# ictnlp/StreamSpeech

Hardware: AMD Instinct MI355X
Metric: real-time factor (RTFx = audio seconds / wall seconds) + utterances/sec, offline S2ST fr-en (higher is better)
Workload: dtype f32

## Files before the change

### include/streamspeech_hip.h

```cpp
#ifndef STREAMSPEECH_HIP_H
#define STREAMSPEECH_HIP_H

#include <stddef.h>
#include <stdint.h>

#ifdef __cplusplus
extern "C" {
#endif

#define SS_ABI_VERSION 2

typedef struct ss_model ss_model;
typedef struct ss_vocoder ss_vocoder;
typedef struct ss_scratch ss_scratch;
typedef struct ss_stream_pool ss_stream_pool;

typedef struct ss_config {
  int32_t input_feat, conv_channels, conv_kernel;
  int32_t enc_dim, enc_ffn, enc_heads, enc_layers, dw_kernel;
  int32_t src_vocab, tgt_vocab;
  int32_t mt_layers, dec_dim, dec_ffn, dec_heads;
  int32_t t2u_layers, unit_layers, unit_vocab, ctc_upsample;
  int32_t pad, eos, unk;
  int32_t max_rel_pos;
// ... 416 lines not shown
                 double* h_bytes_total);
int ss_prof_totals(int cls, double* h_flops_total, double* h_bytes_total, int64_t* h_launches);
int ss_prof_read_issued(int cls, double* h_issued_flops_total);
int ss_prof_shape_log(int on);
int ss_prof_shape_dump(char* buf, int cap);
int ss_prof_num_classes(void);
const char* ss_prof_class_name(int cls);

int ss_model_set_pack_invariant(ss_model* m, int on);
int ss_model_get_pack_invariant(ss_model* m);
int ss_debug_canon(int mode);

int ss_debug_last_logits(ss_model* m, void* stream, float* d_out, int64_t cap_floats, int* h_rows, int* h_cols);

int ss_op_ffn_fused(void* stream, const float* dX, int ldx, float* dY, int ldy, const float* ln_g, const float* ln_b,
                    const float* dW1, const float* db1, const float* dW2, const float* db2, float alpha,
                    const float* ln2_g, const float* ln2_b, int M, int D, int F);
int ss_debug_ffn(int grid, int row_tiles_per_wave, int enable);
int ss_debug_rtlin(int grid, int enable);
int ss_debug_rtlin_kb(int uw, int order);
int ss_debug_rtlin_kb_last(int32_t out[4]);
int ss_debug_conv_c64(int enable);
int ss_debug_conv_c256_rows(int rows);
int ss_debug_conv_c32(int enable);
int ss_debug_conv_c16(int enable);
int64_t ss_debug_enc_step_launches(void);
int ss_op_ln_linear(void* stream, const float* dX, int ldx, const float* ln_g, const float* ln_b, const float* dW,
                    const float* dbias, const float* dR, int ldr, float* dC, int ldc, int M, int N, int K, int act, float alpha,
                    int glu);
int ss_op_ln_linear_ex(void* stream, const float* dX, int ldx, const float* ln_g, const float* ln_b, float* ln_out, const float* dW,
                       const float* dbias, const float* dR, int ldr, float* dC, int ldc, int M, int N, int K, int act, float alpha,
                       int glu, int canon);

int ss_debug_force_tile(int bm, int bn, int ks);
int ss_debug_sk_errors(void);
int ss_debug_attention_split(int v);
int ss_debug_attention_q16(int v);
int ss_debug_enc_step_inject_timeout(ss_model* m);
int ss_debug_scratch_audit(ss_scratch* sc, size_t* booked, size_t* held);
int ss_debug_mt_inject_timeout(ss_model* m);

int ss_op_conv_gemm(void* stream, const float* dA, int lda, const float* dW, const float* dbias,
                    const float* dR, int ldr, const float* dR2, int ldr2, float* dC, int ldc,
                    int M, int N, int Cin, int taps, int dil, int stride, int pad, int in_len,
                    int chunk, int in_act, float in_slope, int act, float alpha, float div, int glu);
typedef struct ss_op_conv_args {
// ... 143 lines not shown
```

### streamspeech_amd/csrc/debug_ops.hip

```cpp
#include "model_internal.hpp"
#include "ctc_align.hpp"

static int op_bind_wino(GemmArgs& a, void* stream) {
  static thread_local std::map<hipStream_t, DevBuf> wino_tmps;
  DevBuf& wino_tmp = wino_tmps[(hipStream_t)stream];
  const int N = a.N, Cin = a.Cin, taps = a.taps;
  if ((conv_c64w_enabled() && N == 64 && Cin == 64 && taps >= 3 && conv_c64_eligible(a)) ||
      (conv_c128w_enabled() && N == 128 && Cin == 128 && taps >= 3 && a.same_rows && !a.glu) ||
      (conv_c256w_enabled() && N == 256 && Cin == 256 && taps >= 3 && a.same_rows && !a.glu) ||
      (conv_c32w_enabled() && N == 32 && Cin == 32 && taps >= 3 && conv_c32_eligible(a))) {
    RET(wino_tmp.ensure((size_t)N * ((taps + 2) / 3) * 4 * N * sizeof(float)));
    RET(launch_wino_pack(a.W, wino_tmp.f(), N, taps, (hipStream_t)stream));
    a.Wwino = wino_tmp.f();
  }
  return SS_OK;
}

extern "C" int ss_op_conv_gemm(void* stream, const float* dA, int lda, const float* dW, const float* dbias,
                               const float* dR, int ldr, const float* dR2, int ldr2, float* dC, int ldc, int M,
                               int N, int Cin, int taps, int dil, int stride, int pad, int in_len, int chunk,
                               int in_act, float in_slope, int act, float alpha, float div, int glu) {
  GemmArgs a;
  a.A = dA; a.lda = lda; a.W = dW; a.bias = dbias; a.R = dR; a.ldr = ldr; a.R2 = dR2; a.ldr2 = ldr2; a.C = dC; a.ldc = ldc;
  a.M = M; a.N = N; a.Cin = Cin; a.taps = taps; a.dil = dil; a.stride = stride; a.pad = pad; a.in_len = in_len;
// ... 95 lines not shown
  a.A = dX; a.lda = ldx; a.W = dW; a.bias = dbias; a.R = dR; a.ldr = ldr; a.C = dC; a.ldc = ldc;
  a.M = M; a.N = N; a.Cin = K; a.in_len = M; a.act = act; a.alpha = alpha; a.glu = glu; a.same_rows = 1;
  a.ln_g = ln_g; a.ln_b = ln_b;
  return launch_conv_gemm(a, (hipStream_t)stream);
}
extern "C" int ss_op_ln_linear_ex(void* stream, const float* dX, int ldx, const float* ln_g, const float* ln_b, float* ln_out,
                                  const float* dW, const float* dbias, const float* dR, int ldr, float* dC, int ldc, int M, int N, int K,
                                  int act, float alpha, int glu, int canon) {
  if (canon < 0 || canon > 2 || (ln_g == nullptr) != (ln_b == nullptr) || (ln_out && !ln_g)) return SS_ERR_ARG;
  GemmArgs a;
  a.A = dX; a.lda = ldx; a.W = dW; a.bias = dbias; a.R = dR; a.ldr = ldr; a.C = dC; a.ldc = ldc;
  a.M = M; a.N = N; a.Cin = K; a.in_len = M; a.act = act; a.alpha = alpha; a.glu = glu; a.same_rows = 1;
  a.ln_g = ln_g; a.ln_b = ln_b; a.ln_out = ln_out; a.canon = canon;
  return launch_conv_gemm(a, (hipStream_t)stream);
}
extern "C" int ss_debug_conv_c64(int enable) {
  if (enable == 4 || enable == 5) { conv_c64w_debug(enable == 5); return SS_OK; }
  if (enable == 6 || enable == 7) { conv_c128w_debug(enable == 7); return SS_OK; }
  if (enable == 8 || enable == 9) { conv_c256w_debug(enable == 9); return SS_OK; }
  conv_c64_debug(enable);
  return SS_OK;
}
extern "C" int ss_debug_conv_c256_rows(int rows) { return conv_c256w_rows_debug(rows); }
extern "C" int ss_debug_conv_c32(int enable) {
  if (enable == 4 || enable == 5) { conv_c32w_debug(enable == 5); return SS_OK; }
  conv_c32_debug(enable);
  return SS_OK;
}
extern "C" int ss_debug_conv_c16(int enable) { conv_c16_debug(enable); return SS_OK; }
extern "C" int64_t ss_debug_enc_step_launches(void) { return (int64_t)enc_step_launch_count(); }
extern "C" int ss_debug_scratch_audit(ss_scratch* sc, size_t* booked, size_t* held) {
  if (!sc || !booked || !held) return SS_ERR_ARG;
  size_t sum = 0;
  bool foreign = false;
  for (DevBuf* b : sc->all()) {
    sum += b->bytes;
    if (b->acct != &sc->acct) foreign = true;
  }
  *booked = sc->acct.used;
  *held = sum;
  return foreign ? SS_ERR_ARG : SS_OK;
}
extern "C" int ss_debug_rtlin(int grid, int enable) {
  if (grid < 0) return SS_ERR_ARG;
  rtlin_debug(grid, enable);
  return SS_OK;
// ... 211 lines not shown
```

### streamspeech_amd/csrc/dispatch.hip

```cpp
#include "gemm.hpp"

#include <atomic>
#include <cstdlib>
#include <map>
#include <mutex>
#include <utility>
#include <vector>

namespace ss {

namespace {
std::mutex g_disp_mu;
std::atomic<unsigned> g_disp_gen{1};
Dispatch env_defaults() {
  Dispatch d;
  auto I = [](const char* k, int dflt) { const char* e = getenv(k); return e ? atoi(e) : dflt; };
  auto L = [](const char* k, long long dflt) { const char* e = getenv(k); return e ? atoll(e) : dflt; };
  d.attn_split = I("SS_ATTN_NO_SPLIT", 0) ? -1 : 0; d.attn_q16 = I("SS_ATTN_Q16", d.attn_q16);
  d.c16_off = I("SS_NO_CONV_C16", 0) ? 1 : 0; d.c32_off = I("SS_NO_CONV_C32", 0) ? 1 : 0; d.c64_off = I("SS_NO_CONV_C64", 0) ? 1 : 0;
  d.c16_min_rows = L("SS_CONV_C16_MIN_ROWS", d.c16_min_rows); d.c32_min_rows = L("SS_CONV_C32_MIN_ROWS", d.c32_min_rows);
  d.c64_min_rows = L("SS_CONV_C64_MIN_ROWS", d.c64_min_rows);
  d.c64w_on = I("SS_CONV_C64_WINOGRAD", 1); d.c128w_on = I("SS_CONV_C128_WINOGRAD", 1); d.c256w_on = I("SS_CONV_C256_WINOGRAD", 1);
  d.c32w_on = I("SS_CONV_C32_WINOGRAD", 1); d.c64w_min_k = I("SS_CONV_C64_WINOGRAD_MIN_K", 3);
  d.c128w_min_rows = L("SS_CONV_C128_MIN_ROWS", d.c128w_min_rows); d.c256w_min_rows = L("SS_CONV_C256_MIN_ROWS", d.c256w_min_rows);
  if (const int r = I("SS_CONV_C256_ROWS", d.c256w_rows); r == 128 || r == 256) d.c256w_rows = r;
  if (getenv("SS_FFN_WM")) { d.ffn_wm = I("SS_FFN_WM", 3); d.ffn_wm_forced = 1; d.ffn_wm_env = d.ffn_wm; }
  d.ffn_fusion = I("SS_NO_FFN_FUSION", 0) ? 0 : 1; d.ffn_min_rows = I("SS_FFN_MIN_ROWS", d.ffn_min_rows);
  if (getenv("SS_SK_MIN_GFLOP")) d.sk_min_flops = 1e9 * atof(getenv("SS_SK_MIN_GFLOP"));
  d.no_resblock_fusion = I("SS_NO_RESBLOCK_FUSION", 0); d.no_pair_fusion = I("SS_NO_PAIR_FUSION", 0);
  d.rt_off = I("SS_NO_RTLIN", 0) ? 1 : 0; d.rt_min_rows = I("SS_RTLIN_MIN_ROWS", d.rt_min_rows); d.rt_min_units = L("SS_RTLIN_MIN_UNITS", d.rt_min_units);
  d.rt_kb_min_units = L("SS_RTLIN_KB_MIN_UNITS", d.rt_kb_min_units); d.rt_kb_uw = I("SS_RTLIN_KB_UW", d.rt_kb_uw); d.rt_kb_xmap = I("SS_RTLIN_KB_XMAP", d.rt_kb_xmap);
  d.smallm_max_rows = I("SS_SMALLM_MAX_ROWS", d.smallm_max_rows); d.sk_min_units = L("SS_SK_MIN_UNITS", d.sk_min_units);
  d.no_sk2 = I("SS_NO_SK2", 0) ? 1 : 0; d.sk2_min_k64 = I("SS_SK2_MINK64", d.sk2_min_k64); d.sk2_spare_cus = I("SS_SK2_SPARE_CUS", 0);
  d.rt_wg_per_cu = I("SS_RTLIN_WG_PER_CU", 0); d.c32_min_k = I("SS_CONV_C32_MIN_K", d.c32_min_k); d.c16_min_k = I("SS_CONV_C16_MIN_K", d.c16_min_k);
  return d;
}
Dispatch& process_settings() { static Dispatch d = env_defaults(); return d; }
thread_local const Dispatch* t_disp = nullptr;
thread_local CtxDispatch t_disp_own;
}
void dispatch_edit(const std::function<void(Dispatch&)>& fn) {
  std::lock_guard<std::mutex> lk(g_disp_mu);
  fn(process_settings());
  g_disp_gen.fetch_add(1, std::memory_order_release);
}
void slab_debug(int grid, long long min_rows) {
  const Dispatch dflt = env_defaults();
  dispatch_edit([=](Dispatch& d) {
    d.slab_grid_cap = grid > 0 ? grid : 0;
    const bool set = min_rows >= 0;
    d.c16_min_rows = set ? min_rows : dflt.c16_min_rows; d.c32_min_rows = set ? min_rows : dflt.c32_min_rows;
    d.c64_min_rows = set ? min_rows : dflt.c64_min_rows;
    d.c128w_min_rows = set ? min_rows : dflt.c128w_min_rows; d.c256w_min_rows = set ? min_rows : dflt.c256w_min_rows;
  });
}
int conv_c256w_rows_debug(int rows) {
  if (rows != 0 && rows != 128 && rows != 256) return SS_ERR_ARG;
  const int dflt = env_defaults().c256w_rows;
  dispatch_edit([=](Dispatch& d) { d.c256w_rows = rows ? rows : dflt; });
  return SS_OK;
}
const Dispatch* CtxDispatch::refresh() {
  const unsigned now = g_disp_gen.load(std::memory_order_acquire);
  if (gen != now) {
    std::lock_guard<std::mutex> lk(g_disp_mu);
    d = process_settings();
    gen = g_disp_gen.load(std::memory_order_relaxed);
  }
  return &d;
}
const Dispatch& disp() { return t_disp ? *t_disp : *t_disp_own.refresh(); }
DispatchScope::DispatchScope(const Dispatch* d) : prev(t_disp) { t_disp = d; }
DispatchScope::~DispatchScope() { t_disp = prev; }

void debug_force_tile(int bm, int bn, int ks) {
  dispatch_edit([=](Dispatch& d) { d.force_bm = bm; d.force_bn = bn; d.force_ks = ks; d.sk_groups = (bm == 1 && bn == 8); });
}
bool debug_tile_forced() { return disp().force_bm != 0; }

static thread_local int t_canon = CANON_NONE;
CanonScope::CanonScope(int mode) : prev(t_canon) { t_canon = mode; }
CanonScope::~CanonScope() { t_canon = prev; }
// ... 93 lines not shown
```

### streamspeech_amd/csrc/dispatch.hpp

```cpp
#pragma once
#include <functional>

namespace ss {

struct Dispatch {
  int attn_no_mfma = 0;
  int attn_q16 = 1;
  int attn_split = 0;
  int c16_off = 0, c32_off = 0, c64_off = 0;
  long long c16_min_rows = 131072, c32_min_rows = 65536, c64_min_rows = 32768;
  int c64w_on = 1, c128w_on = 1, c256w_on = 1, c32w_on = 1;
  int c64w_min_k = 3;
  long long c128w_min_rows = 65536, c256w_min_rows = 32768;
  int c256w_rows = 128;
  int c32_min_k = 7, c16_min_k = 11;
  int slab_grid_cap = 0;
  int sk_groups = 0;
  int sk2_spare_cus = 0;
  int ffn_force_g = 0;
  int ffn_wm = 3, ffn_wm_forced = 0;
  int ffn_wm_env = 0;
  int ffn_fusion = 1;
  int ffn_min_rows = 1000;
  int force_bm = 0, force_bn = 0, force_ks = 0;
  double sk_min_flops = 4e9;
  int smallm_max_rows = 192;
  long long sk_min_units = 12 * 512;
  int no_sk2 = 0;
  int sk2_min_k64 = 192;
  int no_resblock_fusion = 0, no_pair_fusion = 0;
  int rt_off = 0, rt_min_rows = 193, rt_force_g = 0;
  long long rt_min_units = 4000;
  int rt_wg_per_cu = 0;
  long long rt_kb_min_units = 256;
  int rt_kb_xmap = 1;
  int rt_kb_uw = 0;
  int rt_kb_order = 1;
};

const Dispatch& disp();
void dispatch_edit(const std::function<void(Dispatch&)>& fn);

struct CtxDispatch {
  Dispatch d;
  unsigned gen = 0xffffffffu;
  const Dispatch* refresh();
};
struct DispatchScope {
  explicit DispatchScope(const Dispatch* d);
// ... 6 lines not shown
```

### streamspeech_amd/csrc/gemm.hip

```cpp
#include "gemm.hpp"

#include <type_traits>

namespace ss {

using f32x4 = __attribute__((ext_vector_type(4))) float;

template <int BM, int BN, int BK, int WM, int WN, int KS, int PD, bool BLK = false>
__global__ __launch_bounds__(256 * KS) void conv_gemm_kernel(const GemmArgs p) {
  static_assert(WM * WN == 4, "4 waves per k-group");
  static_assert(!BLK || KS == 1, "the blocked chain is the KS = 1 form");
  constexpr int LDK = BK + 8;
  constexpr int WTM = BM / WM, WTN = BN / WN;
  constexpr int TM = WTM / 16, TN = WTN / 16;
  static_assert(TM >= 1 && TN >= 1, "wave tile must hold a 16x16 MFMA tile");
  constexpr int KQ = BK / 4;
  constexpr int A_F4 = BM * KQ, W_F4 = BN * KQ;
  constexpr int NA = (A_F4 + 255) / 256, NW = (W_F4 + 255) / 256;
  constexpr int STAGE = (BM + BN) * LDK;
  extern __shared__ __attribute__((aligned(16))) float smem_all[];
  const int kg = threadIdx.x >> 8;
  float* smem = smem_all + kg * 2 * STAGE;

  const int t = threadIdx.x & 255, lane = t & 63, wave = t >> 6;
// ... 269 lines not shown
          if (p.R2) x = p.R2[row * p.ldr2 + n + e] + x;
          if (p.div > 0.f) x = x / p.div;
          p.C[row * p.ldc + n + e] = x;
          if (p.C2) p.C2[row * p.ldc2 + n + e] = x > 0.f ? x : x * p.c2_slope;
        }
      }
    }
  }
}


__device__ __forceinline__ void linear_store(const GemmArgs& p, int m, int n, float acc, float b) {
  float v = acc + b;
  switch (p.act) {
    case ACT_SILU: v = v / (1.0f + expf(-v)); break;
    case ACT_RELU: v = fmaxf(v, 0.f); break;
    default: break;
  }
  v *= p.alpha;
  if (p.R) v += p.R[(size_t)m * p.ldr + n];
  p.C[(size_t)m * p.ldc + n] = v;
}

template <int SK, int WN, bool LNORM, bool GLU = false>
__global__ __launch_bounds__(256) void smallm_gemm_kernel(const GemmArgs p) {
  static_assert(SK * WN == 4, "4 waves");
  static_assert(!GLU || (SK == 2 && WN == 2), "GLU: wave column 0 = the 16 value columns, 1 = the 16 gate columns of a 32-column block");
  __shared__ f32x4 red[SK > 1 ? (SK - 1) * WN * 64 : 1];
  __shared__ float ln_stat[32];
  const int t = threadIdx.x, lane = t & 63, wave = t >> 6;
  const int sk = wave / WN, wn = wave % WN;
  const int r = lane & 15, g = lane >> 4;
  if ((int)blockIdx.x * (16 * WN) >= p.N) return;
  const int m0 = blockIdx.y * 16;
  const int n0 = blockIdx.x * (16 * WN) + wn * 16;
  const int K = p.Cin;
  const int KC = K / 16;
  const int c_begin = (KC * sk) / SK, c_end = (KC * (sk + 1)) / SK;

  const int am = m0 + r;
  const bool a_ok = am < p.M;
  const float* arow = p.A + (size_t)(a_ok ? am : 0) * p.lda + 4 * g;
  const int wnr = n0 + r;
  const bool w_ok = wnr < p.N;
  const float* wrow = p.W + (size_t)(w_ok ? wnr : 0) * K + 4 * g;

  float mean = 0.f, rstd = 1.f;
  if (LNORM) {
    const int lr = t >> 4, part = t & 15;
    const bool ok = (m0 + lr) < p.M;
    const float* xr = p.A + (size_t)(ok ? m0 + lr : 0) * p.lda + part * 4;
    f32x4 v[8];
    float sm = 0.f;
#pragma unroll
    for (int j = 0; j < 8; ++j) {
      v[j] = f32x4{0.f, 0.f, 0.f, 0.f};
      if (j * 64 < K && ok) v[j] = *reinterpret_cast<const f32x4*>(xr + j * 64);
      sm += (v[j][0] + v[j][1]) + (v[j][2] + v[j][3]);
    }
#pragma unroll
    for (int o = 1; o < 16; o <<= 1) sm += __shfl_xor(sm, o, 64);
    const float mu = sm / (float)K;
    float q = 0.f;
#pragma unroll
    for (int j = 0; j < 8; ++j)
      if (j * 64 < K) {
#pragma unroll
        for (int e = 0; e < 4; ++e) { const float d = v[j][e] - mu; q += d * d; }
      }
#pragma unroll
    for (int o = 1; o < 16; o <<= 1) q += __shfl_xor(q, o, 64);
    if (part == 0) { ln_stat[lr] = mu; ln_stat[16 + lr] = 1.0f / sqrtf(q / (float)K + 1e-5f); }
    __syncthreads();
    mean = ln_stat[r];
    rstd = ln_stat[16 + r];
  }

  f32x4 acc = {0.f, 0.f, 0.f, 0.f}, acc2 = {0.f, 0.f, 0.f, 0.f};
  f32x4 tot = {0.f, 0.f, 0.f, 0.f};
  const bool blocked = (c_end - c_begin) > 8;
  auto load4 = [&](f32x4 (&a)[4], f32x4 (&w)[4], int c) {
#pragma unroll
    for (int u = 0; u < 4; ++u) {
      a[u] = f32x4{0.f, 0.f, 0.f, 0.f};
      w[u] = f32x4{0.f, 0.f, 0.f, 0.f};
      if (a_ok) a[u] = *reinterpret_cast<const f32x4*>(arow + (c + u) * 16);
      if (w_ok) w[u] = *reinterpret_cast<const f32x4*>(wrow + (c + u) * 16);
    }
  };
  auto mma = [&](f32x4 a, f32x4 w, int c) {
    if (LNORM) {
      const f32x4 gm = *reinterpret_cast<const f32x4*>(p.ln_g + c * 16 + 4 * g);
      const f32x4 bt = *reinterpret_cast<const f32x4*>(p.ln_b + c * 16 + 4 * g);
#pragma unroll
      for (int e = 0; e < 4; ++e) a[e] = a_ok ? (a[e] - mean) * rstd * gm[e] + bt[e] : 0.f;
    }
    acc = __builtin_amdgcn_mfma_f32_16x16x4f32(a[0], w[0], acc, 0, 0, 0);
    acc2 = __builtin_amdgcn_mfma_f32_16x16x4f32(a[1], w[1], acc2, 0, 0, 0);
    acc = __builtin_amdgcn_mfma_f32_16x16x4f32(a[2], w[2], acc, 0, 0, 0);
    acc2 = __builtin_amdgcn_mfma_f32_16x16x4f32(a[3], w[3], acc2, 0, 0, 0);
    if (blocked && (c & 3) == 3) {
#pragma unroll
      for (int e = 0; e < 4; ++e) { tot[e] += acc[e] + acc2[e]; acc[e] = 0.f; acc2[e] = 0.f; }
    }
  };
  auto mma4 = [&](f32x4 (&a)[4], f32x4 (&w)[4], int c) {
#pragma unroll
    for (int u = 0; u < 4; ++u) mma(a[u], w[u], c + u);
  };
  const int G = (c_end - c_begin) / 4;
  f32x4 a0[4], w0[4], a1[4], w1[4];
  if (G > 0) load4(a0, w0, c_begin);
  for (int gi = 0; gi < G; gi += 2) {
    const int c = c_begin + 4 * gi;
    if (gi + 1 < G) load4(a1, w1, c + 4);
    mma4(a0, w0, c);
    if (gi + 1 < G) {
      if (gi + 2 < G) load4(a0, w0, c + 8);
      mma4(a1, w1, c + 4);
    }
  }
  for (int c = c_begin + 4 * G; c < c_end; ++c) {
    f32x4 a = {0.f, 0.f, 0.f, 0.f}, w = {0.f, 0.f, 0.f, 0.f};
    if (a_ok) a = *reinterpret_cast<const f32x4*>(arow + c * 16);
    if (w_ok) w = *reinterpret_cast<const f32x4*>(wrow + c * 16);
    mma(a, w, c);
  }
#pragma unroll
  for (int e = 0; e < 4; ++e) acc[e] = tot[e] + (acc[e] + acc2[e]);

  if (SK > 1) {
    if (sk > 0) red[((sk - 1) * WN + wn) * 64 + lane] = acc;
    __syncthreads();
    if (!GLU && sk > 0) return;
    if (sk == 0) {
#pragma unroll
      for (int s2 = 1; s2 < SK; ++s2) {
        const f32x4 o = red[((s2 - 1) * WN + wn) * 64 + lane];
#pragma unroll
        for (int e = 0; e < 4; ++e) acc[e] += o[e];
      }
    }
  }
  if constexpr (GLU) {
    __shared__ f32x4 gate_tile[64];
    const int ncol = n0 + r;
    const float bcol = (p.bias && ncol < p.N) ? p.bias[ncol] : 0.f;
    if (sk == 0 && wn == 1) {
      f32x4 gt;
#pragma unroll
      for (int e = 0; e < 4; ++e) gt[e] = acc[e] + bcol;
      gate_tile[lane] = gt;
    }
    __syncthreads();
    if (sk != 0 || wn != 0 || ncol + 16 >= p.N) return;
    const f32x4 gt = gate_tile[lane];
    const int oc = (int)blockIdx.x * 16 + r;
#pragma unroll
    for (int e = 0; e < 4; ++e) {
      const int m = m0 + g * 4 + e;
      if (m < p.M) p.C[(size_t)m * p.ldc + oc] = (acc[e] + bcol) * (1.0f / (1.0f + expf(-gt[e])));
    }
    return;
  }
  const int n = n0 + r;
  if (n >= p.N) return;
  const float b = p.bias ? p.bias[n] : 0.f;
#pragma unroll
  for (int e = 0; e < 4; ++e) {
    const int m = m0 + g * 4 + e;
    if (m < p.M) linear_store(p, m, n, acc[e], b);
  }
}


template <int MR, int KS, bool LNORM>
__global__ __launch_bounds__(256) void gemv_kernel(const GemmArgs p) {
  constexpr int WPB = 4;
  constexpr int CPB = WPB / KS;
  __shared__ float part[WPB][MR];
  const int t = threadIdx.x, lane = t & 63, wave = t >> 6;
  const int col = blockIdx.x * CPB + wave / KS;
  const int ks = wave % KS;
  const int K = p.Cin;
  const int kper = K / KS;
  const int k0 = ks * kper;
  const int nit = kper / 256;
  const bool col_ok = col < p.N;

  f32x4 wv[8];
  const float* wrow = p.W + (size_t)(col_ok ? col : 0) * K + k0 + 4 * lane;
#pragma unroll
  for (int it = 0; it < 8; ++it) {
    wv[it] = f32x4{0.f, 0.f, 0.f, 0.f};
    if (it < nit && col_ok) wv[it] = *reinterpret_cast<const f32x4*>(wrow + it * 256);
// ... 95 lines not shown
  static_assert((size_t)(KS - 1) * BM * BN * sizeof(float) <= kLds, "reduction scratch fits the staging buffers");
  if constexpr (kLds > 64 * 1024) SS_MAX_LDS_ONCE((&conv_gemm_kernel<BM, BN, BK, WM, WN, KS, PD, BLK>), kLds);
  const int mmax = (a.nseg > 0 ? a.max_seg_out : a.M) - a.m_begin;
  dim3 grid(cdiv(mmax, BM), cdiv(a.N, BN), a.nseg > 0 ? a.nseg : 1);
  if (grid.x >= 32 && grid.y * grid.z > 1) grid.x = (grid.x + 7) & ~7u;
  ProfRec rec{}; bool prof = false;
  int rc = prof_begin(a, stream, cls, rec, prof);
  if (rc != SS_OK) return rc;
  hipLaunchKernelGGL((conv_gemm_kernel<BM, BN, BK, WM, WN, KS, PD, BLK>), grid, dim3(256 * KS), kLds, stream, a);
  SS_LAUNCH_CHECK();
  return prof_end(stream, rec, prof);
}

template <int BM, int BN, int BK, int WM, int WN, int MAXKS>
static int launch_cfg_ks(const GemmArgs& a, hipStream_t stream, ProfCls cls, long tiles) {
  const int nk = a.taps * (a.Cin / BK);
  int ks = 1;
  while (ks < MAXKS && tiles * 4 * ks < 1024 && nk / (ks * 2) >= 2) ks *= 2;
  if constexpr (MAXKS >= 4) { if (ks >= 4) return launch_cfg<BM, BN, BK, WM, WN, 4>(a, stream, cls); }
  if constexpr (MAXKS >= 2) { if (ks >= 2) return launch_cfg<BM, BN, BK, WM, WN, 2>(a, stream, cls); }
  return launch_cfg<BM, BN, BK, WM, WN, 1>(a, stream, cls);
}

template <int SK, int WN, bool GLU = false>
static int launch_smallm(const GemmArgs& a, hipStream_t stream, ProfCls cls) {
  if (a.ln_g && a.Cin > 512) return SS_ERR_ARG;
  dim3 grid((cdiv(a.N, 16 * WN) + 7) & ~7, cdiv(a.M, 16));
  ProfRec rec{}; bool prof = false;
  int rc = prof_begin(a, stream, cls, rec, prof);
  if (rc != SS_OK) return rc;
  if (a.ln_g) hipLaunchKernelGGL((smallm_gemm_kernel<SK, WN, true, GLU>), grid, dim3(256), 0, stream, a);
  else hipLaunchKernelGGL((smallm_gemm_kernel<SK, WN, false, GLU>), grid, dim3(256), 0, stream, a);
  SS_LAUNCH_CHECK();
  return prof_end(stream, rec, prof);
}


template <bool BLK, int BM, int BN, int BK, int WM, int WN, int MAXKS>
static int launch_rung(const GemmArgs& a, hipStream_t stream, ProfCls cls, long tiles) {
  if constexpr (BLK) return launch_cfg<BM, BN, BK, WM, WN, 1, 1, true>(a, stream, cls);
  else return launch_cfg_ks<BM, BN, BK, WM, WN, MAXKS>(a, stream, cls, tiles);
}

template <bool BLK>
static int launch_32x64(const GemmArgs& a, hipStream_t stream, long tiles) {
  if (a.Cin % 32 != 0) return launch_rung<BLK, 32, 64, 16, 2, 2, 4>(a, stream, PROF_GEMM_32x64x16, tiles);
  if (tiles >= 768) return launch_rung<BLK, 32, 64, 32, 2, 2, 1>(a, stream, PROF_GEMM_32x64x32, tiles);
  return launch_rung<BLK, 32, 64, 32, 2, 2, 4>(a, stream, PROF_GEMM_32x64x32, tiles);
}

template <bool BLK>
static int launch_tiles(const GemmArgs& a, hipStream_t stream, int M, int nseg) {
  const bool k32 = (a.Cin % 32) == 0;
  const long t128 = (long)cdiv(M, 128) * nseg;
  if (a.N <= 16) return launch_rung<BLK, 128, 16, 16, 4, 1, 2>(a, stream, PROF_GEMM_128x16x16, t128);
// ... 115 lines not shown
```

### streamspeech_amd/csrc/gemm.hpp

```cpp
#pragma once
#include "common.hpp"
#include "dispatch.hpp"
#include "prof.hpp"

namespace ss {

struct GemmArgs {
  const float* A = nullptr;
  const float* W = nullptr;
  const float* Wwino = nullptr;
  const void* Wf16 = nullptr;
  const float* bias = nullptr;
  const float* R = nullptr;
  const float* R2 = nullptr;
  float* C = nullptr;
  int lda = 0, ldc = 0, ldr = 0, ldr2 = 0;
  int M = 0, N = 0, Cin = 0;
  int taps = 1, dil = 1, stride = 1, pad = 0;
  int in_len = 0;
  int chunk = 0;
  int m_begin = 0;
  int in_act = ACT_NONE;
  float in_slope = 0.1f;
  int act = ACT_NONE;
// ... 125 lines not shown
int launch_conv_f16(const GemmArgs& a, hipStream_t stream);
size_t f16_pack_halves(int C, int taps);
int launch_f16_pack(const float* W, void* Wf, int C, int taps, hipStream_t stream);

bool rtlin_eligible(const GemmArgs& a);
bool rtlin_shape_ok(const GemmArgs& a);
int launch_rtlin(const GemmArgs& a, hipStream_t stream);
void rtlin_debug(int grid, int enable);
bool rtlin_kb_shape_ok(const GemmArgs& a);
bool rtlin_kb_eligible(const GemmArgs& a);
int launch_rtlin_kb(const GemmArgs& a, hipStream_t stream);
void rtlin_kb_debug(int uw, int order);
void rtlin_kb_last(int out[4]);

bool ffn_fused_eligible(int D, int F, int act, int M, int ldx, int ldy, bool canon = false);
int launch_ffn_fused(const float* X, int ldx, float* Y, int ldy, const float* ln_g, const float* ln_b, const float* W1,
                     const float* b1, const float* W2, const float* b2, float alpha, const float* ln2_g, const float* ln2_b,
                     int M, int D, int F, hipStream_t stream, int canon = 0);
void ffn_fused_debug_grid(int g);
void ffn_fused_debug_rows(int wm);

bool gemv_eligible(const GemmArgs& a);
bool smallm_eligible(const GemmArgs& a);

void debug_force_tile(int bm, int bn, int ks);
bool debug_tile_forced();

int launch_conv_gemm(const GemmArgs& a, hipStream_t stream);

}
```

### streamspeech_amd/lib.py

```python
import ctypes as C
import os

_HERE = os.path.dirname(os.path.abspath(__file__))
LIB_PATH = os.environ.get("SS_HIP_LIB") or os.path.join(_HERE, "libstreamspeech_hip.so")


class SSConfig(C.Structure):
    _fields_ = [(n, C.c_int32) for n in (
        "input_feat", "conv_channels", "conv_kernel", "enc_dim", "enc_ffn", "enc_heads", "enc_layers",
        "dw_kernel", "src_vocab", "tgt_vocab", "mt_layers", "dec_dim", "dec_ffn", "dec_heads",
        "t2u_layers", "unit_layers", "unit_vocab", "ctc_upsample", "pad", "eos", "unk",
        "max_rel_pos", "max_tgt_pos")]


class SSVocoderConfig(C.Structure):
    _fields_ = [
        ("num_embeddings", C.c_int32), ("embedding_dim", C.c_int32), ("model_in_dim", C.c_int32),
        ("upsample_initial_channel", C.c_int32),
        ("n_up", C.c_int32), ("upsample_rates", C.c_int32 * 8), ("upsample_kernel_sizes", C.c_int32 * 8),
        ("n_res", C.c_int32), ("resblock_kernel_sizes", C.c_int32 * 4), ("resblock_dilations", (C.c_int32 * 3) * 4),
        ("dur_hidden", C.c_int32), ("dur_kernel", C.c_int32)]


_vp, _i, _f, _i64 = C.c_void_p, C.c_int, C.c_float, C.c_int64
# ... 252 lines not shown
                                 C.POINTER(C.c_int32), _vp, _vp, _vp, _vp]),
    "ss_unit_spans_host": (_i, [_i, _vp, C.POINTER(C.c_int32), C.POINTER(C.c_int32), C.POINTER(C.c_int32), C.POINTER(C.c_int32), _vp,
                                _i, _i, _i, _i, _i, _vp, _vp]),
    "ss_op_unit_spans": (_i, [_vp, _i, _vp, C.POINTER(C.c_int32), C.POINTER(C.c_int32), C.POINTER(C.c_int32), C.POINTER(C.c_int32),
                              _vp, _i, _i, _i, _i, _i, _vp, _vp]),
    "ss_prof_enable": (_i, [_i]),
    "ss_prof_enable_hi": (_i, [_i]),
    "ss_prof_reset": (_i, []),
    "ss_prof_read": (_i, [_i, C.POINTER(C.c_double), C.POINTER(C.c_double), C.POINTER(_i64), C.POINTER(C.c_double)]),
    "ss_prof_totals": (_i, [_i, C.POINTER(C.c_double), C.POINTER(C.c_double), C.POINTER(_i64)]),
    "ss_prof_read_issued": (_i, [_i, C.POINTER(C.c_double)]),
    "ss_prof_shape_log": (_i, [_i]),
    "ss_prof_shape_dump": (_i, [C.c_char_p, _i]),
    "ss_prof_num_classes": (_i, []),
    "ss_prof_class_name": (C.c_char_p, [_i]),
    "ss_debug_force_tile": (_i, [_i, _i, _i]),
    "ss_op_ffn_fused": (_i, [_vp, _vp, _i, _vp, _i, _vp, _vp, _vp, _vp, _vp, _vp, _f, _vp, _vp, _i, _i, _i]),
    "ss_debug_ffn": (_i, [_i, _i, _i]),
    "ss_debug_rtlin": (_i, [_i, _i]),
    "ss_debug_rtlin_kb": (_i, [_i, _i]),
    "ss_debug_rtlin_kb_last": (_i, [C.POINTER(C.c_int32)]),
    "ss_debug_conv_c64": (_i, [_i]),
    "ss_debug_conv_c256_rows": (_i, [_i]),
    "ss_debug_conv_c32": (_i, [_i]),
    "ss_debug_conv_c16": (_i, [_i]),
    "ss_debug_enc_step_launches": (_i64, []),
    "ss_debug_scratch_audit": (_i, [_vp, C.POINTER(C.c_size_t), C.POINTER(C.c_size_t)]),
    "ss_op_ln_linear": (_i, [_vp, _vp, _i, _vp, _vp, _vp, _vp, _vp, _i, _vp, _i, _i, _i, _i, _i, _f, _i]),
    "ss_op_ln_linear_ex": (_i, [_vp, _vp, _i, _vp, _vp, _vp, _vp, _vp, _vp, _i, _vp, _i, _i, _i, _i, _i, _f, _i, _i]),
    "ss_debug_last_logits": (_i, [_vp, _vp, _vp, _i64, C.POINTER(_i), C.POINTER(_i)]),
    "ss_debug_sk_errors": (_i, []),
    "ss_debug_attention_split": (_i, [_i]),
    "ss_debug_attention_q16": (_i, [_i]),
    "ss_op_conv_gemm": (_i, [_vp, _vp, _i, _vp, _vp, _vp, _i, _vp, _i, _vp, _i, _i, _i, _i, _i, _i, _i, _i, _i, _i,
                             _i, _f, _i, _f, _f, _i]),
    "ss_op_conv_gemm_ex": (_i, [_vp, C.POINTER(SSOpConvArgs)]),
    "ss_op_conv_gemm_rows": (_i, [_vp, C.POINTER(SSOpConvArgs), _i, _vp, _vp, _i]),
    "ss_op_conv_pair": (_i, [_vp, _vp, _i, _vp, _vp, _vp, _vp, _vp, _i, _vp, _i, _f, _vp, _i, _f, _i, _i, _i, _i, _i, _f, _vp, _i]),
    "ss_op_resblock_fused": (_i, [_vp, _vp, _i, _vp, _vp, _vp, _vp, _vp, _vp, _i, _vp, _i, _f, _i, _i, _i, _f, _vp, _i]),
    "ss_debug_slab": (_i, [_i, C.c_longlong]),
    "ss_op_conv_f16": (_i, [_vp, _vp, _vp, _vp, _vp, _vp, _vp, _vp, _i, _i, _i, _i, _i, _f, _i, _f, _vp, _i]),
    "ss_op_layernorm": (_i, [_vp, _vp, _i, _vp, _i, _vp, _vp, _i, _i, _f]),
    "ss_op_attention": (_i, [_vp, _vp, _i, _vp, _i, _vp, _i, _vp, _i, _i, _i, _i, _f, _i, _i, _vp, _i, _vp, _vp]),
    "ss_op_attention_ex": (_i, [_vp, C.POINTER(SSOpAttnArgs)]),
    "ss_op_attention_probs": (_i, [_vp, C.POINTER(SSOpAttnProbsArgs)]),
    "ss_op_attention_pool": (_i, [_vp, C.POINTER(SSOpPoolAttnArgs)]),
# ... 79 lines not shown
```

Baseline: 6418.

## Add multi-row-tile small-M GEMM variant reusing weight loads across row tiles

Templates the small-M MFMA GEMM kernel on a row-tile count so each workgroup can process 2 or 4 sixteen-row tiles while loading each weight fragment once, reducing weight traffic when the grid is large relative to CU count. The kernel also preloads LayerNorm gamma/beta per chunk instead of reloading them inside every MMA, restructures the software pipeline, and adds occupancy hints through launch_bounds. A heuristic picks RT=2 for canonical small-M calls when the grid exceeds CUs times the occupancy target, with an env/debug override. The tradeoff is more registers and fewer workgroups, which can lower parallelism.

```diff
diff --git a/include/streamspeech_hip.h b/include/streamspeech_hip.h
--- a/include/streamspeech_hip.h
+++ b/include/streamspeech_hip.h
@@ -462,6 +462,7 @@
 int ss_debug_rtlin_kb_last(int32_t out[4]);
 int ss_debug_conv_c64(int enable);
 int ss_debug_conv_c256_rows(int rows);
+int ss_debug_smallm_rt(int rt);
 int ss_debug_conv_c32(int enable);
 int ss_debug_conv_c16(int enable);
 int64_t ss_debug_enc_step_launches(void);
diff --git a/streamspeech_amd/csrc/debug_ops.hip b/streamspeech_amd/csrc/debug_ops.hip
--- a/streamspeech_amd/csrc/debug_ops.hip
+++ b/streamspeech_amd/csrc/debug_ops.hip
@@ -141,6 +141,7 @@
   return SS_OK;
 }
 extern "C" int ss_debug_conv_c256_rows(int rows) { return conv_c256w_rows_debug(rows); }
+extern "C" int ss_debug_smallm_rt(int rt) { return smallm_rt_debug(rt); }
 extern "C" int ss_debug_conv_c32(int enable) {
   if (enable == 4 || enable == 5) { conv_c32w_debug(enable == 5); return SS_OK; }
   conv_c32_debug(enable);
diff --git a/streamspeech_amd/csrc/dispatch.hip b/streamspeech_amd/csrc/dispatch.hip
--- a/streamspeech_amd/csrc/dispatch.hip
+++ b/streamspeech_amd/csrc/dispatch.hip
@@ -31,6 +31,7 @@
   d.rt_off = I("SS_NO_RTLIN", 0) ? 1 : 0; d.rt_min_rows = I("SS_RTLIN_MIN_ROWS", d.rt_min_rows); d.rt_min_units = L("SS_RTLIN_MIN_UNITS", d.rt_min_units);
   d.rt_kb_min_units = L("SS_RTLIN_KB_MIN_UNITS", d.rt_kb_min_units); d.rt_kb_uw = I("SS_RTLIN_KB_UW", d.rt_kb_uw); d.rt_kb_xmap = I("SS_RTLIN_KB_XMAP", d.rt_kb_xmap);
   d.smallm_max_rows = I("SS_SMALLM_MAX_ROWS", d.smallm_max_rows); d.sk_min_units = L("SS_SK_MIN_UNITS", d.sk_min_units);
+  if (const int rt = I("SS_SMALLM_RT", 0); rt == 1 || rt == 2 || rt == 4) d.smallm_rt = rt;
   d.no_sk2 = I("SS_NO_SK2", 0) ? 1 : 0; d.sk2_min_k64 = I("SS_SK2_MINK64", d.sk2_min_k64); d.sk2_spare_cus = I("SS_SK2_SPARE_CUS", 0);
   d.rt_wg_per_cu = I("SS_RTLIN_WG_PER_CU", 0); d.c32_min_k = I("SS_CONV_C32_MIN_K", d.c32_min_k); d.c16_min_k = I("SS_CONV_C16_MIN_K", d.c16_min_k);
   return d;
@@ -58,6 +59,12 @@
   if (rows != 0 && rows != 128 && rows != 256) return SS_ERR_ARG;
   const int dflt = env_defaults().c256w_rows;
   dispatch_edit([=](Dispatch& d) { d.c256w_rows = rows ? rows : dflt; });
+  return SS_OK;
+}
+int smallm_rt_debug(int rt) {
+  if (rt != 0 && rt != 1 && rt != 2 && rt != 4) return SS_ERR_ARG;
+  const int dflt = env_defaults().smallm_rt;
+  dispatch_edit([=](Dispatch& d) { d.smallm_rt = rt ? rt : dflt; });
   return SS_OK;
 }
 const Dispatch* CtxDispatch::refresh() {
diff --git a/streamspeech_amd/csrc/dispatch.hpp b/streamspeech_amd/csrc/dispatch.hpp
--- a/streamspeech_amd/csrc/dispatch.hpp
+++ b/streamspeech_amd/csrc/dispatch.hpp
@@ -25,6 +25,7 @@
   int force_bm = 0, force_bn = 0, force_ks = 0;
   double sk_min_flops = 4e9;
   int smallm_max_rows = 192;
+  int smallm_rt = 0;
   long long sk_min_units = 12 * 512;
   int no_sk2 = 0;
   int sk2_min_k64 = 192;
diff --git a/streamspeech_amd/csrc/gemm.hip b/streamspeech_amd/csrc/gemm.hip
--- a/streamspeech_amd/csrc/gemm.hip
+++ b/streamspeech_amd/csrc/gemm.hip
@@ -315,124 +315,208 @@
   p.C[(size_t)m * p.ldc + n] = v;
 }
 
-template <int SK, int WN, bool LNORM, bool GLU = false>
-__global__ __launch_bounds__(256) void smallm_gemm_kernel(const GemmArgs p) {
+constexpr int smallm_min_waves(int sk, bool lnorm, int rt) {
+  if (rt == 1) return lnorm ? 3 : 4;
+  if (lnorm && sk == 2) return rt == 4 ? 1 : 2;
+  return rt == 4 ? 2 : 3;
+}
+template <int SK, int WN, bool LNORM, bool GLU = false, int RT = 1>
+__global__ __launch_bounds__(256, smallm_min_waves(SK, LNORM, RT)) void smallm_gemm_kernel(const GemmArgs p) {
   static_assert(SK * WN == 4, "4 waves");
   static_assert(!GLU || (SK == 2 && WN == 2), "GLU: wave column 0 = the 16 value columns, 1 = the 16 gate columns of a 32-column block");
-  __shared__ f32x4 red[SK > 1 ? (SK - 1) * WN * 64 : 1];
-  __shared__ float ln_stat[32];
+  static_assert(RT == 1 || RT == 2 || RT == 4, "row tiles per workgroup");
+  static_assert(!GLU || RT == 1, "the GLU form keeps one row tile");
+  __shared__ f32x4 red[SK > 1 ? (SK - 1) * WN * 64 * RT : 1];
+  __shared__ float ln_stat[32 * RT];
   const int t = threadIdx.x, lane = t & 63, wave = t >> 6;
   const int sk = wave / WN, wn = wave % WN;
   const int r = lane & 15, g = lane >> 4;
   if ((int)blockIdx.x * (16 * WN) >= p.N) return;
-  const int m0 = blockIdx.y * 16;
+  const int m0 = blockIdx.y * (16 * RT);
   const int n0 = blockIdx.x * (16 * WN) + wn * 16;
   const int K = p.Cin;
   const int KC = K / 16;
   const int c_begin = (KC * sk) / SK, c_end = (KC * (sk + 1)) / SK;
-
-  const int am = m0 + r;
-  const bool a_ok = am < p.M;
-  const float* arow = p.A + (size_t)(a_ok ? am : 0) * p.lda + 4 * g;
+  const int nrt = RT == 1 ? 1 : min(RT, (p.M - m0 + 15) / 16);
+
+  bool a_ok[RT];
+  const float* arow[RT];
+#pragma unroll
+  for (int i = 0; i < RT; ++i) {
+    const int am = m0 + 16 * i + r;
+    a_ok[i] = am < p.M;
+    arow[i] = p.A + (size_t)(a_ok[i] ? am : 0) * p.lda + 4 * g;
+  }
   const int wnr = n0 + r;
   const bool w_ok = wnr < p.N;
   const float* wrow = p.W + (size_t)(w_ok ? wnr : 0) * K + 4 * g;
 
-  float mean = 0.f, rstd = 1.f;
+  constexpr int AB = RT == 1 ? 2 : 1;
+  f32x4 a[AB][RT][4], w[2][4], gm[4], bt[4];
+  auto load_w = [&](f32x4 (&wd)[4], int c) {
+#pragma unroll
+    for (int u = 0; u < 4; ++u) {
+      wd[u] = f32x4{0.f, 0.f, 0.f, 0.f};
+      if (w_ok) wd[u] = *reinterpret_cast<const f32x4*>(wrow + (c + u) * 16);
+    }
+  };
+  auto load_a = [&](f32x4 (&ad)[4], int i, int c) {
+#pragma unroll
+    for (int u = 0; u < 4; ++u) {
+      ad[u] = f32x4{0.f, 0.f, 0.f, 0.f};
+      if (a_ok[i]) ad[u] = *reinterpret_cast<const f32x4*>(arow[i] + (c + u) * 16);
+    }
+  };
+  auto load_gb = [&](f32x4 (&gd)[4], f32x4 (&bd)[4], int c) {
+    if (LNORM) {
+#pragma unroll
+      for (int u = 0; u < 4; ++u) {
+        gd[u] = *reinterpret_cast<const f32x4*>(p.ln_g + (c + u) * 16 + 4 * g);
+        bd[u] = *reinterpret_cast<const f32x4*>(p.ln_b + (c + u) * 16 + 4 * g);
+      }
+    }
+  };
+  const int G = (c_end - c_begin) / 4;
+  if (G > 0) {
+    load_w(w[0], c_begin);
+    load_gb(gm, bt, c_begin);
+#pragma unroll
+    for (int i = 0; i < RT; ++i)
+      if (i < nrt) load_a(a[0][i], i, c_begin);
+  }
+
+  float mean[RT], rstd[RT];
+#pragma unroll
+  for (int i = 0; i < RT; ++i) { mean[i] = 0.f; rstd[i] = 1.f; }
   if (LNORM) {
     const int lr = t >> 4, part = t & 15;
-    const bool ok = (m0 + lr) < p.M;
-    const float* xr = p.A + (size_t)(ok ? m0 + lr : 0) * p.lda + part * 4;
-    f32x4 v[8];
-    float sm = 0.f;
-#pragma unroll
-    for (int j = 0; j < 8; ++j) {
-      v[j] = f32x4{0.f, 0.f, 0.f, 0.f};
-      if (j * 64 < K && ok) v[j] = *reinterpret_cast<const f32x4*>(xr + j * 64);
-      sm += (v[j][0] + v[j][1]) + (v[j][2] + v[j][3]);
-    }
-#pragma unroll
-    for (int o = 1; o < 16; o <<= 1) sm += __shfl_xor(sm, o, 64);
-    const float mu = sm / (float)K;
-    float q = 0.f;
-#pragma unroll
-    for (int j = 0; j < 8; ++j)
-      if (j * 64 < K) {
-#pragma unroll
-        for (int e = 0; e < 4; ++e) { const float d = v[j][e] - mu; q += d * d; }
-      }
-#pragma unroll
-    for (int o = 1; o < 16; o <<= 1) q += __shfl_xor(q, o, 64);
-    if (part == 0) { ln_stat[lr] = mu; ln_stat[16 + lr] = 1.0f / sqrtf(q / (float)K + 1e-5f); }
+#pragma unroll
+    for (int i = 0; i < RT; ++i) {
+      if (i >= nrt) continue;
+      const int row = m0 + 16 * i + lr;
+      const bool ok = row < p.M;
+      const float* xr = p.A + (size_t)(ok ? row : 0) * p.lda + part * 4;
+      f32x4 v[8];
+      float sm = 0.f;
+#pragma unroll
+      for (int j = 0; j < 8; ++j) {
+        v[j] = f32x4{0.f, 0.f, 0.f, 0.f};
+        if (j * 64 < K && ok) v[j] = *reinterpret_cast<const f32x4*>(xr + j * 64);
+        sm += (v[j][0] + v[j][1]) + (v[j][2] + v[j][3]);
+      }
+#pragma unroll
+      for (int o = 1; o < 16; o <<= 1) sm += __shfl_xor(sm, o, 64);
+      const float mu = sm / (float)K;
+      float q = 0.f;
+#pragma unroll
+      for (int j = 0; j < 8; ++j)
+        if (j * 64 < K) {
+#pragma unroll
+          for (int e = 0; e < 4; ++e) { const float d = v[j][e] - mu; q += d * d; }
+        }
+#pragma unroll
+      for (int o = 1; o < 16; o <<= 1) q += __shfl_xor(q, o, 64);
+      if (part == 0) { ln_stat[32 * i + lr] = mu; ln_stat[32 * i + 16 + lr] = 1.0f / sqrtf(q / (float)K + 1e-5f); }
+    }
     __syncthreads();
-    mean = ln_stat[r];
-    rstd = ln_stat[16 + r];
-  }
-
-  f32x4 acc = {0.f, 0.f, 0.f, 0.f}, acc2 = {0.f, 0.f, 0.f, 0.f};
-  f32x4 tot = {0.f, 0.f, 0.f, 0.f};
-  const bool blocked = (c_end - c_begin) > 8;
-  auto load4 = [&](f32x4 (&a)[4], f32x4 (&w)[4], int c) {
-#pragma unroll
-    for (int u = 0; u < 4; ++u) {
-      a[u] = f32x4{0.f, 0.f, 0.f, 0.f};
-      w[u] = f32x4{0.f, 0.f, 0.f, 0.f};
-      if (a_ok) a[u] = *reinterpret_cast<const f32x4*>(arow + (c + u) * 16);
-      if (w_ok) w[u] = *reinterpret_cast<const f32x4*>(wrow + (c + u) * 16);
-    }
+#pragma unroll
+    for (int i = 0; i < RT; ++i)
+      if (i < nrt) { mean[i] = ln_stat[32 * i + r]; rstd[i] = ln_stat[32 * i + 16 + r]; }
+  }
+
+  f32x4 acc[RT], acc2[RT], tot[RT];
+#pragma unroll
+  for (int i = 0; i < RT; ++i) { acc[i] = f32x4{0.f, 0.f, 0.f, 0.f}; acc2[i] = f32x4{0.f, 0.f, 0.f, 0.f}; tot[i] = f32x4{0.f, 0.f, 0.f, 0.f}; }
+  const bool blocked = !(LNORM && SK == 4) && (c_end - c_begin) > 8;
+  auto norm = [&](f32x4& x, const f32x4& gd, const f32x4& bd, int i) {
+#pragma unroll
+    for (int e = 0; e < 4; ++e) x[e] = a_ok[i] ? (x[e] - mean[i]) * rstd[i] * gd[e] + bd[e] : 0.f;
   };
-  auto mma = [&](f32x4 a, f32x4 w, int c) {
-    if (LNORM) {
-      const f32x4 gm = *reinterpret_cast<const f32x4*>(p.ln_g + c * 16 + 4 * g);
-      const f32x4 bt = *reinterpret_cast<const f32x4*>(p.ln_b + c * 16 + 4 * g);
-#pragma unroll
-      for (int e = 0; e < 4; ++e) a[e] = a_ok ? (a[e] - mean) * rstd * gm[e] + bt[e] : 0.f;
-    }
-    acc = __builtin_amdgcn_mfma_f32_16x16x4f32(a[0], w[0], acc, 0, 0, 0);
-    acc2 = __builtin_amdgcn_mfma_f32_16x16x4f32(a[1], w[1], acc2, 0, 0, 0);
-    acc = __builtin_amdgcn_mfma_f32_16x16x4f32(a[2], w[2], acc, 0, 0, 0);
-    acc2 = __builtin_amdgcn_mfma_f32_16x16x4f32(a[3], w[3], acc2, 0, 0, 0);
+  auto mma = [&](int i, const f32x4& x, const f32x4& wv, int c) {
+    acc[i] = __builtin_amdgcn_mfma_f32_16x16x4f32(x[0], wv[0], acc[i], 0, 0, 0);
+    acc2[i] = __builtin_amdgcn_mfma_f32_16x16x4f32(x[1], wv[1], acc2[i], 0, 0, 0);
+    acc[i] = __builtin_amdgcn_mfma_f32_16x16x4f32(x[2], wv[2], acc[i], 0, 0, 0);
+    acc2[i] = __builtin_amdgcn_mfma_f32_16x16x4f32(x[3], wv[3], acc2[i], 0, 0, 0);
     if (blocked && (c & 3) == 3) {
 #pragma unroll
-      for (int e = 0; e < 4; ++e) { tot[e] += acc[e] + acc2[e]; acc[e] = 0.f; acc2[e] = 0.f; }
+      for (int e = 0; e < 4; ++e) { tot[i][e] += acc[i][e] + acc2[i][e]; acc[i][e] = 0.f; acc2[i][e] = 0.f; }
     }
   };
-  auto mma4 = [&](f32x4 (&a)[4], f32x4 (&w)[4], int c) {
-#pragma unroll
-    for (int u = 0; u < 4; ++u) mma(a[u], w[u], c + u);
+  auto step = [&](auto bsel, int c, bool more) {
+    constexpr int b = decltype(bsel)::value, ab = b & (AB - 1), an = (b ^ 1) & (AB - 1);
+    if constexpr (RT == 1) {
+      if (more) { load_w(w[b ^ 1], c + 4); load_a(a[an][0], 0, c + 4); }
+      if (LNORM) {
+#pragma unroll
+        for (int u = 0; u < 4; ++u) norm(a[ab][0][u], gm[u], bt[u], 0);
+        if (more) load_gb(gm, bt, c + 4);
+      }
+#pragma unroll
+      for (int u = 0; u < 4; ++u) mma(0, a[ab][0][u], w[b][u], c + u);
+    } else {
+      if (LNORM) {
+#pragma unroll
+        for (int i = 0; i < RT; ++i)
+          if (i < nrt) {
+#pragma unroll
+            for (int u = 0; u < 4; ++u) norm(a[0][i][u], gm[u], bt[u], i);
+          }
+      }
+      if (more) { load_w(w[b ^ 1], c + 4); load_gb(gm, bt, c + 4); }
+#pragma unroll
+      for (int i = 0; i < RT; ++i)
+        if (i < nrt) {
+#pragma unroll
+          for (int u = 0; u < 4; ++u) mma(i, a[0][i][u], w[b][u], c + u);
+          if (more) load_a(a[0][i], i, c + 4);
+        }
+    }
   };
-  const int G = (c_end - c_begin) / 4;
-  f32x4 a0[4], w0[4], a1[4], w1[4];
-  if (G > 0) load4(a0, w0, c_begin);
   for (int gi = 0; gi < G; gi += 2) {
     const int c = c_begin + 4 * gi;
-    if (gi + 1 < G) load4(a1, w1, c + 4);
-    mma4(a0, w0, c);
-    if (gi + 1 < G) {
-      if (gi + 2 < G) load4(a0, w0, c + 8);
-      mma4(a1, w1, c + 4);
-    }
+    step(std::integral_constant<int, 0>{}, c, gi + 1 < G);
+    if (gi + 1 < G) step(std::integral_constant<int, 1>{}, c + 4, gi + 2 < G);
   }
   for (int c = c_begin + 4 * G; c < c_end; ++c) {
-    f32x4 a = {0.f, 0.f, 0.f, 0.f}, w = {0.f, 0.f, 0.f, 0.f};
-    if (a_ok) a = *reinterpret_cast<const f32x4*>(arow + c * 16);
-    if (w_ok) w = *reinterpret_cast<const f32x4*>(wrow + c * 16);
-    mma(a, w, c);
-  }
-#pragma unroll
-  for (int e = 0; e < 4; ++e) acc[e] = tot[e] + (acc[e] + acc2[e]);
+    f32x4 wv = {0.f, 0.f, 0.f, 0.f}, gd = {0.f, 0.f, 0.f, 0.f}, bd = {0.f, 0.f, 0.f, 0.f};
+    if (w_ok) wv = *reinterpret_cast<const f32x4*>(wrow + c * 16);
+    if (LNORM) {
+      gd = *reinterpret_cast<const f32x4*>(p.ln_g + c * 16 + 4 * g);
+      bd = *reinterpret_cast<const f32x4*>(p.ln_b + c * 16 + 4 * g);
+    }
+#pragma unroll
+    for (int i = 0; i < RT; ++i)
+      if (i < nrt) {
+        f32x4 x = {0.f, 0.f, 0.f, 0.f};
+        if (a_ok[i]) x = *reinterpret_cast<const f32x4*>(arow[i] + c * 16);
+        if (LNORM) norm(x, gd, bd, i);
+        mma(i, x, wv, c);
+      }
+  }
+#pragma unroll
+  for (int i = 0; i < RT; ++i)
+#pragma unroll
+    for (int e = 0; e < 4; ++e) acc[i][e] = tot[i][e] + (acc[i][e] + acc2[i][e]);
 
   if (SK > 1) {
-    if (sk > 0) red[((sk - 1) * WN + wn) * 64 + lane] = acc;
+    if (sk > 0) {
+#pragma unroll
+      for (int i = 0; i < RT; ++i)
+        if (i < nrt) red[(((sk - 1) * WN + wn) * RT + i) * 64 + lane] = acc[i];
+    }
     __syncthreads();
     if (!GLU && sk > 0) return;
     if (sk == 0) {
 #pragma unroll
-      for (int s2 = 1; s2 < SK; ++s2) {
-        const f32x4 o = red[((s2 - 1) * WN + wn) * 64 + lane];
-#pragma unroll
-        for (int e = 0; e < 4; ++e) acc[e] += o[e];
-      }
+      for (int i = 0; i < RT; ++i)
+        if (i < nrt) {
+#pragma unroll
+          for (int s2 = 1; s2 < SK; ++s2) {
+            const f32x4 o = red[(((s2 - 1) * WN + wn) * RT + i) * 64 + lane];
+#pragma unroll
+            for (int e = 0; e < 4; ++e) acc[i][e] += o[e];
+          }
+        }
     }
   }
   if constexpr (GLU) {
@@ -442,7 +526,7 @@
     if (sk == 0 && wn == 1) {
       f32x4 gt;
 #pragma unroll
-      for (int e = 0; e < 4; ++e) gt[e] = acc[e] + bcol;
+      for (int e = 0; e < 4; ++e) gt[e] = acc[0][e] + bcol;
       gate_tile[lane] = gt;
     }
     __syncthreads();
@@ -452,7 +536,7 @@
 #pragma unroll
     for (int e = 0; e < 4; ++e) {
       const int m = m0 + g * 4 + e;
-      if (m < p.M) p.C[(size_t)m * p.ldc + oc] = (acc[e] + bcol) * (1.0f / (1.0f + expf(-gt[e])));
+      if (m < p.M) p.C[(size_t)m * p.ldc + oc] = (acc[0][e] + bcol) * (1.0f / (1.0f + expf(-gt[e])));
     }
     return;
   }
@@ -460,10 +544,12 @@
   if (n >= p.N) return;
   const float b = p.bias ? p.bias[n] : 0.f;
 #pragma unroll
-  for (int e = 0; e < 4; ++e) {
-    const int m = m0 + g * 4 + e;
-    if (m < p.M) linear_store(p, m, n, acc[e], b);
-  }
+  for (int i = 0; i < RT; ++i)
+#pragma unroll
+    for (int e = 0; e < 4; ++e) {
+      const int m = m0 + 16 * i + g * 4 + e;
+      if (m < p.M) linear_store(p, m, n, acc[i][e], b);
+    }
 }
 
 
@@ -605,15 +691,39 @@
   return launch_cfg<BM, BN, BK, WM, WN, 1>(a, stream, cls);
 }
 
+static int smallm_rt(const GemmArgs& a, int sk, int wn) {
+  const int forced = disp().smallm_rt;
+  if (forced == 1 || forced == 2 || forced == 4) return forced;
+  if (a.canon != CANON_SMALLM || a.M <= 16 || (a.ln_g && sk == 2)) return 1;
+  const int ncg = (cdiv(a.N, 16 * wn) + 7) & ~7;
+  if (ncg <= 32) return 1;
+  int cus = 0;
+  if (device_cus(cus) != SS_OK) return 1;
+  return (long)ncg * cdiv(a.M, 16) > (long)cus * smallm_min_waves(sk, a.ln_g != nullptr, 1) ? 2 : 1;
+}
+
+template <int SK, int WN, bool GLU, int RT>
+static void launch_smallm_rt(const GemmArgs& a, hipStream_t stream) {
+  dim3 grid((cdiv(a.N, 16 * WN) + 7) & ~7, cdiv(a.M, 16 * RT));
+  if (a.ln_g) hipLaunchKernelGGL((smallm_gemm_kernel<SK, WN, true, GLU, RT>), grid, dim3(256), 0, stream, a);
+  else hipLaunchKernelGGL((smallm_gemm_kernel<SK, WN, false, GLU, RT>), grid, dim3(256), 0, stream, a);
+}
+
 template <int SK, int WN, bool GLU = false>
 static int launch_smallm(const GemmArgs& a, hipStream_t stream, ProfCls cls) {
   if (a.ln_g && a.Cin > 512) return SS_ERR_ARG;
-  dim3 grid((cdiv(a.N, 16 * WN) + 7) & ~7, cdiv(a.M, 16));
+  int rt = 1;
+  if constexpr (!GLU && SK > 1) rt = smallm_rt(a, SK, WN);
   ProfRec rec{}; bool prof = false;
   int rc = prof_begin(a, stream, cls, rec, prof);
   if (rc != SS_OK) return rc;
-  if (a.ln_g) hipLaunchKernelGGL((smallm_gemm_kernel<SK, WN, true, GLU>), grid, dim3(256), 0, stream, a);
-  else hipLaunchKernelGGL((smallm_gemm_kernel<SK, WN, false, GLU>), grid, dim3(256), 0, stream, a);
+  if constexpr (!GLU && SK > 1) {
+    if (rt == 4) launch_smallm_rt<SK, WN, GLU, 4>(a, stream);
+    else if (rt == 2) launch_smallm_rt<SK, WN, GLU, 2>(a, stream);
+    else launch_smallm_rt<SK, WN, GLU, 1>(a, stream);
+  } else {
+    launch_smallm_rt<SK, WN, GLU, 1>(a, stream);
+  }
   SS_LAUNCH_CHECK();
   return prof_end(stream, rec, prof);
 }
diff --git a/streamspeech_amd/csrc/gemm.hpp b/streamspeech_amd/csrc/gemm.hpp
--- a/streamspeech_amd/csrc/gemm.hpp
+++ b/streamspeech_amd/csrc/gemm.hpp
@@ -171,6 +171,7 @@
 
 bool gemv_eligible(const GemmArgs& a);
 bool smallm_eligible(const GemmArgs& a);
+int smallm_rt_debug(int rt);
 
 void debug_force_tile(int bm, int bn, int ks);
 bool debug_tile_forced();
diff --git a/streamspeech_amd/lib.py b/streamspeech_amd/lib.py
--- a/streamspeech_amd/lib.py
+++ b/streamspeech_amd/lib.py
@@ -298,6 +298,7 @@
     "ss_debug_rtlin_kb_last": (_i, [C.POINTER(C.c_int32)]),
     "ss_debug_conv_c64": (_i, [_i]),
     "ss_debug_conv_c256_rows": (_i, [_i]),
+    "ss_debug_smallm_rt": (_i, [_i]),
     "ss_debug_conv_c32": (_i, [_i]),
     "ss_debug_conv_c16": (_i, [_i]),
     "ss_debug_enc_step_launches": (_i64, []),
```

After: 6457, median of 6. About the same (+0.6%).
